# lunarlab-gatech/SLIDE_SLAM

Hardware: AMD Instinct MI355X
Metric: pose-graph updates/sec + ms/Gauss-Newton iter, 8-robot 10k-landmark graph (higher is better)
Workload: dtype f64

## Files before the change

### slide_slam_amd/csrc/chol_kernels.hip

```cpp
#include <hip/hip_runtime.h>
#include <stdlib.h>
#include <algorithm>
#include <type_traits>
#include <utility>
#include <vector>

#include "graph_dev.hpp"
#include "kernels.hpp"

namespace sl {

typedef double v4d __attribute__((ext_vector_type(4)));
constexpr int CHOL_BATCH_MAX = 8;
__device__ inline v4d mfma_f64(double a, double b, v4d c) { return __builtin_amdgcn_mfma_f64_16x16x4f64(a, b, c, 0, 0, 0); }

__device__ inline double rsqrt_nr(double d) {
#ifdef SLIDE_RSQRT_OLD
  double y = __builtin_amdgcn_rsq(d);
  y = y * (1.5 - 0.5 * d * y * y);
  y = y * (1.5 - 0.5 * d * y * y);
  return y;
#else
  double y = __builtin_amdgcn_rsq(d);
  double t = d * y, h = 0.5 * y;
// ... 2182 lines not shown
    if (tid < NB) ys[row] = r0 - ((red[0][row] + red[1][row]) + (red[2][row] + red[3][row]));
  } else {
    acc += __shfl_xor(acc, 1);
    acc += __shfl_xor(acc, 2);
    if (worker && part == 0) ys[i] = r0 - acc;
  }
  __syncthreads();
  if (!worker && has_p) poll(FWD ? c - 1 : c + 1, nloop & 1);
  double z = 0.0;
#pragma unroll
  for (int k = 0; k < 16; ++k) z += mt[k] * ys[16 * part + k];
  z += __shfl_xor(z, 1);
  z += __shfl_xor(z, 2);
  if (has_p) {
    __syncthreads();
    double pv = 0.0;
#pragma unroll
    for (int k = 0; k < 16; ++k) pv += pt[k] * xs[nloop & 1][16 * part + k];
    pv += __shfl_xor(pv, 1);
    pv += __shfl_xor(pv, 2);
    z -= pv;
  }
  if (worker && part == 0) __hip_atomic_store(xout + (size_t)c * NB + i, z, __ATOMIC_RELAXED, __HIP_MEMORY_SCOPE_AGENT);
}
struct ChainBatchArgs {
  int n;
  const double* S[CHOL_BATCH_MAX]; int ld[CHOL_BATCH_MAX]; int T[CHOL_BATCH_MAX];
  const double* ctab[CHOL_BATCH_MAX]; const double* in[CHOL_BATCH_MAX]; double* out[CHOL_BATCH_MAX];
  int* status[CHOL_BATCH_MAX];
  const float* L32[CHOL_BATCH_MAX];
  const int* prof[CHOL_BATCH_MAX];
  const int* first[CHOL_BATCH_MAX];
  double* next_out[CHOL_BATCH_MAX];
  int* next_ticket;
  int Tmax;
};
template <bool FWD, bool F32>
__global__ __launch_bounds__(CHAIN_THREADS) void k_chain_batched(ChainBatchArgs A) {
  __shared__ TabLds W;
  for (;;) {
    const int t = bwd_ticket(&A.status[0][FWD ? 5 : 4]);
    if (t >= A.n * A.Tmax) return;
    const int r = t % A.n, b = t / A.n;
    if (t == 0 && A.next_ticket && threadIdx.x == 0) *A.next_ticket = 0;
    if (b >= A.T[r]) continue;
    tab_chain_body<FWD, F32>(W, A.S[r], A.ld[r], A.T[r], A.L32[r], A.ctab[r], A.in[r], A.out[r], A.status[r], FWD ? b : A.T[r] - 1 - b,
                             A.prof[r], A.first[r], A.next_out[r]);
    return;
  }
}
struct ChainPrepArgs { int n; double* out[CHOL_BATCH_MAX]; int len[CHOL_BATCH_MAX]; int* ticket; };
__global__ void k_chain_prepare(ChainPrepArgs A) {
  const int r = blockIdx.y;
  const int i = blockIdx.x * blockDim.x + threadIdx.x;
  if (r == 0 && i == 0) *A.ticket = 0;
  if (i < A.len[r]) A.out[r][i] = __longlong_as_double((long long)BWD_SENT);
}
static bool chain_has_tables(const CholSystem* d, int n) {
  for (int i = 0; i < n; ++i)
    if (!d[i].L32 || !d[i].ctab) return false;
  return n > 0;
}
void launch_chain_tables(const CholSystem* d, int n, hipStream_t s) {
  if (!chain_has_tables(d, n)) return;
  ChainTabArgs A{};
  A.n = n;
  int Tmax = 0;
  for (int i = 0; i < n; ++i) {
    A.T[i] = d[i].T; A.S[i] = d[i].S; A.ld[i] = d[i].ld; A.Ld[i] = d[i].Ld; A.Winv[i] = d[i].Winv; A.prof[i] = d[i].prof; A.ctab[i] = d[i].ctab;
    Tmax = d[i].T > Tmax ? d[i].T : Tmax;
  }
  if (Tmax > 0) hipLaunchKernelGGL(k_chain_tables, dim3(Tmax, n), dim3(256), 0, s, A);
}
void launch_chain_batch(const CholSystem* d, int n, const double* const* in, double* const* out, bool fwd, bool f32, bool prepared,
                        double* const* next_out, hipStream_t s) {
  ChainBatchArgs A{};
  ChainPrepArgs Pr{};
  A.n = n;
  Pr.n = n;
  int Tmax = 0, total = 0;
  for (int i = 0; i < n; ++i) {
    A.S[i] = d[i].S; A.ld[i] = d[i].ld; A.T[i] = d[i].T; A.ctab[i] = d[i].ctab; A.in[i] = in[i]; A.out[i] = out[i];
    A.status[i] = d[i].status;
    A.L32[i] = d[i].L32;
    A.prof[i] = d[i].prof; A.first[i] = d[i].first;
    Tmax = d[i].T > Tmax ? d[i].T : Tmax;
    total += d[i].T;
    Pr.out[i] = out[i];
    Pr.len[i] = d[i].T * NB;
    A.next_out[i] = next_out ? next_out[i] : nullptr;
  }
  A.next_ticket = next_out ? d[0].status + (fwd ? 4 : 5) : nullptr;
  A.Tmax = Tmax;
  if (total <= 0) return;
  if (!chain_has_tables(d, n)) { fprintf(stderr, "slide_slam_amd: launch_chain_batch without the tables / the packed f32 factor\n"); abort(); }
  Pr.ticket = d[0].status + (fwd ? 5 : 4);
  if (!prepared) hipLaunchKernelGGL(k_chain_prepare, dim3((Tmax * NB + 255) / 256, n), dim3(256), 0, s, Pr);
  if (fwd) {
    if (f32) hipLaunchKernelGGL((k_chain_batched<true, true>), dim3(total), dim3(CHAIN_THREADS), 0, s, A);
    else hipLaunchKernelGGL((k_chain_batched<true, false>), dim3(total), dim3(CHAIN_THREADS), 0, s, A);
  } else {
    if (f32) hipLaunchKernelGGL((k_chain_batched<false, true>), dim3(total), dim3(CHAIN_THREADS), 0, s, A);
    else hipLaunchKernelGGL((k_chain_batched<false, false>), dim3(total), dim3(CHAIN_THREADS), 0, s, A);
  }
}

__global__ __launch_bounds__(256) void k_cov_fwd(const double* __restrict__ S, int ld, int k, const double* __restrict__ Ldk,
                                                 const double* __restrict__ Wk, double* __restrict__ Y, int nT) {
  __shared__ double yk[6][NB];
  __shared__ double xk[6][NB];
  const int tid = threadIdx.x;
  for (int e = tid; e < 6 * NB; e += 256) yk[e / NB][e % NB] = Y[(size_t)(e / NB) * nT + (size_t)k * NB + e % NB];
  __syncthreads();
  const int c = tid >> 4, r = tid & 15;
#pragma unroll 1
  for (int b = 0; b < 4; ++b) {
    if (c < 6) {
      double s = 0.0;
#pragma unroll
      for (int j = 0; j < 16; ++j) s += Wk[(size_t)b * 256 + j * 16 + r] * yk[c][16 * b + j];
      xk[c][16 * b + r] = s;
    }
    __syncthreads();
    for (int e = tid; e < 6 * 16 * (3 - b); e += 256) {
      const int cc = e / (16 * (3 - b)), m = 16 * (b + 1) + e % (16 * (3 - b));
      double s = 0.0;
#pragma unroll
      for (int n = 0; n < 16; ++n) s += Ldk[(size_t)(16 * b + n) * NB + m] * xk[cc][16 * b + n];
      yk[cc][m] -= s;
    }
    __syncthreads();
  }
  if (blockIdx.x == 0) {
    for (int e = tid; e < 6 * NB; e += 256) Y[(size_t)(e / NB) * nT + (size_t)k * NB + e % NB] = xk[e / NB][e % NB];
    return;
  }
  const int i = k + (int)blockIdx.x;
  const double* tile = S + (size_t)(k * NB) * ld + (size_t)i * NB;
  for (int e = tid; e < 6 * NB; e += 256) {
    const int cc = e / NB, row = e % NB;
    double s = 0.0;
#pragma unroll 8
    for (int q = 0; q < NB; ++q) s += tile[(size_t)q * ld + row] * xk[cc][q];
    Y[(size_t)cc * nT + (size_t)i * NB + row] -= s;
  }
}
__global__ __launch_bounds__(256) void k_cov_gram(const double* __restrict__ Y, int nT, int row0, double* __restrict__ cov36) {
  __shared__ double part[36][257];
  const int tid = threadIdx.x;
  double acc[36];
#pragma unroll
  for (int e = 0; e < 36; ++e) acc[e] = 0.0;
  for (int row = row0 + tid; row < nT; row += 256) {
    double y[6];
#pragma unroll
    for (int c = 0; c < 6; ++c) y[c] = Y[(size_t)c * nT + row];
#pragma unroll
    for (int a = 0; a < 6; ++a)
#pragma unroll
      for (int b = 0; b < 6; ++b) acc[6 * a + b] += y[a] * y[b];
  }
#pragma unroll
  for (int e = 0; e < 36; ++e) part[e][tid] = acc[e];
  __syncthreads();
  if (tid < 36) {
    double s = 0.0;
    for (int q = 0; q < 256; ++q) s += part[tid][q];
    cov36[tid] = s;
  }
}
void launch_pose_covariance(const double* S, int ld, int T, const double* Ld, const double* Winv, double* Y, int row0, double* cov36,
                            hipStream_t s) {
  const int nT = T * NB;
  for (int k = row0 / NB; k < T; ++k)
    hipLaunchKernelGGL(k_cov_fwd, dim3((unsigned)(T - k)), dim3(256), 0, s, S, ld, k, Ld + (size_t)k * NB * NB, Winv + (size_t)k * 1024, Y, nT);
  hipLaunchKernelGGL(k_cov_gram, dim3(1), dim3(256), 0, s, Y, nT, row0 / NB * NB, cov36);
}

struct SyrkArgs {
  int n;
  const double* S[CHOL_BATCH_MAX]; int ld[CHOL_BATCH_MAX]; int T[CHOL_BATCH_MAX]; int nbr[CHOL_BATCH_MAX];
  int b0[CHOL_BATCH_MAX];
  double* bord[CHOL_BATCH_MAX]; int ldb[CHOL_BATCH_MAX]; const int* bfirst[CHOL_BATCH_MAX];
  const double* bsrc[CHOL_BATCH_MAX];
  int ks; double* scratch;
  size_t scratch_stride;
  int ks_sys[4];
  double* scratch2; size_t scratch_stride2;
  const int* jobs;
  const int* segtab[CHOL_BATCH_MAX];
};
template <int RD>
__device__ __forceinline__ void border_syrk_body(const SyrkArgs& A) {
  int r = A.ks > 1 ? 0 : blockIdx.z, ib = blockIdx.x, jb = blockIdx.y;
  const int q = A.ks > 1 ? blockIdx.z : 0;
  if (A.jobs) {
    const int j = A.jobs[blockIdx.x];
    r = j >> 20; ib = (j >> 10) & 1023; jb = j & 1023;
  }
  const int nbr = A.nbr[r];
  if (ib > nbr || jb >= nbr || ib < jb) return;
  const int T = A.T[r], ld = A.ld[r];
  int ldb = A.ldb[r];
  int c0 = 0, c1 = T;
  const int* st = A.segtab[r];
  const int nseg = st ? st[0] : 1;
  if (!st && A.bfirst[r]) c0 = max(A.bfirst[r][ib], A.bfirst[r][jb]);
  int ksr = A.ks;
  if (A.ks > 1) {
    if (A.scratch_stride && r < 4 && A.ks_sys[r] > 0) ksr = A.ks_sys[r];
    if (q >= ksr) return;
    const int len = (T - c0 + ksr - 1) / ksr;
    c0 += q * len;
    c1 = min(T, c0 + len);
  }
  const double* bsrc = A.bsrc[r];
  if (!st && c0 >= c1 && !(bsrc && q == 0)) return;
  const double* S = A.S[r];
  const int wq = threadIdx.x >> 6, lane = threadIdx.x & 63, lr = lane & 15, lk = lane >> 4;
  const int ch = (wq >> 1) & 1, rh = wq & 1;
  if (A.jobs && ib == nbr && rh == 1 && !bsrc) return;
  const int B0 = A.b0[r];
  const double* pj0 = S + (size_t)lk * ld + (size_t)(B0 + jb) * NB + 32 * ch + 2 * lr;
  const double* pi0 = S + (size_t)lk * ld + (size_t)(B0 + ib) * NB + 32 * rh + 2 * lr;
  double* cbh = A.bord[r] + (size_t)(jb * NB + 32 * ch + 2 * lk) * ldb + (size_t)ib * NB + 32 * rh + 2 * lr;
  const double* cin = bsrc ? bsrc + (size_t)(jb * NB + 32 * ch + 2 * lk) * ldb + (size_t)ib * NB + 32 * rh + 2 * lr : cbh;
  const int ldin = ldb;
  if (q > 0) {
    ldb = NB;
    double* sc = r < 2 ? A.scratch + (size_t)r * A.scratch_stride : A.scratch2 + (size_t)(r - 2) * A.scratch_stride2;
    cbh = sc + ((size_t)(jb * (nbr + 1) + ib) * (ksr - 1) + (q - 1)) * (NB * NB) + (size_t)(32 * ch + 2 * lk) * NB + 32 * rh + 2 * lr;
  }
  int total = 0;
  if (st) {
    for (int sg = 0; sg < nseg; ++sg) {
      const int* sf = st + 1 + nseg + sg * (nbr + 1);
      const int a0 = max(sf[ib], sf[jb]), a1 = st[1 + sg];
      if (a0 < a1) total += (a1 - a0) * 16;
    }
  } else {
    total = c1 > c0 ? (c1 - c0) * 16 : 0;
  }
  int sg_next = 0, rem = 0, issued = 0;
  const double *lpj = pj0, *lpi = pi0;
  v2d pa[RD], pb[RD];
  auto issue = [&](v2d& ra, v2d& rb) {
    while (rem == 0 && sg_next < nseg) {
      int a0 = c0, a1 = c1;
      if (st) {
        const int* sf = st + 1 + nseg + sg_next * (nbr + 1);
        a0 = max(sf[ib], sf[jb]);
        a1 = st[1 + sg_next];
      }
      ++sg_next;
      if (a0 < a1) {
        rem = (a1 - a0) * 16;
        lpj = pj0 + (size_t)a0 * NB * ld;
        lpi = pi0 + (size_t)a0 * NB * ld;
      }
    }
    ra = *(const v2d*)lpj;
    rb = *(const v2d*)lpi;
    lpj += (size_t)4 * ld;
    lpi += (size_t)4 * ld;
    --rem;
    ++issued;
  };
#pragma unroll
  for (int pre = 0; pre < RD - 1; ++pre)
    if (issued < total) issue(pa[pre], pb[pre]);
  v4d acc[2][2];
#pragma unroll
  for (int a = 0; a < 2; ++a)
#pragma unroll
    for (int e = 0; e < 4; ++e) {
      v2d c2;
      c2[0] = 0.0; c2[1] = 0.0;
      if (q == 0) c2 = *(const v2d*)(cin + (size_t)(8 * e + a) * ldin);
      acc[a][0][e] = c2[0]; acc[a][1][e] = c2[1];
    }
  for (int ks0 = 0; ks0 < total; ks0 += RD) {
#pragma unroll
    for (int u = 0; u < RD; ++u) {
      if (issued < total) issue(pa[(u + RD - 1) % RD], pb[(u + RD - 1) % RD]);
      __builtin_amdgcn_sched_barrier(0);
#pragma unroll
      for (int a = 0; a < 2; ++a) {
        const double na = -pa[u][a];
#pragma unroll
        for (int b = 0; b < 2; ++b) acc[a][b] = mfma_f64(na, pb[u][b], acc[a][b]);
      }
      __builtin_amdgcn_sched_barrier(0);
    }
  }
#pragma unroll
  for (int a = 0; a < 2; ++a)
#pragma unroll
    for (int e = 0; e < 4; ++e) {
      v2d c2;
      c2[0] = acc[a][0][e]; c2[1] = acc[a][1][e];
      *(v2d*)(cbh + (size_t)(8 * e + a) * ldb) = c2;
    }
}
__global__ __launch_bounds__(256) void k_border_syrk(SyrkArgs A) { border_syrk_body<16>(A); }
__global__ __launch_bounds__(256) void k_border_syrk_rd8(SyrkArgs A) { border_syrk_body<8>(A); }
__global__ __launch_bounds__(256) void k_border_syrk_rd4(SyrkArgs A) { border_syrk_body<4>(A); }
static void launch_syrk_kernel(dim3 grid, size_t lds, hipStream_t s, const SyrkArgs& A) {
  static const int rd = getenv("SLIDE_SYRK_RD") ? atoi(getenv("SLIDE_SYRK_RD")) : 16;
  if (rd == 4) hipLaunchKernelGGL(k_border_syrk_rd4, grid, dim3(256), lds, s, A);
  else if (rd == 8) hipLaunchKernelGGL(k_border_syrk_rd8, grid, dim3(256), lds, s, A);
  else hipLaunchKernelGGL(k_border_syrk, grid, dim3(256), lds, s, A);
}
template <int N>
__device__ __forceinline__ void border_reduce_elems(double* __restrict__ bord, int ldb, int nbr, int ks, const double* __restrict__ scratch,
                                                    const int* __restrict__ bfirst, int T, int ib, int jb, int e0, int stride) {
  if (ib > nbr || jb >= nbr || ib < jb) return;
  int c0 = 0;
  if (bfirst) c0 = max(bfirst[ib], bfirst[jb]);
  const int len = (T - c0 + ks - 1) / ks;
  double* dst[N];
  double v[N];
#pragma unroll
  for (int u = 0; u < N; ++u) {
    const int e = e0 + u * stride;
    const int col = e / NB, row = e - col * NB;
    dst[u] = bord + (size_t)(jb * NB + col) * ldb + (size_t)ib * NB + row;
    v[u] = *dst[u];
  }
  int nq = ks;
  while (nq > 1 && c0 + (nq - 1) * len >= T) --nq;
  const double* sq = scratch + (size_t)(jb * (nbr + 1) + ib) * (ks - 1) * (NB * NB) + e0;
  int q = 1;
  for (; q + 1 < nq; q += 2) {
    double p[N], p2[N];
#pragma unroll
    for (int u = 0; u < N; ++u) { p[u] = sq[(size_t)(q - 1) * (NB * NB) + u * stride]; p2[u] = sq[(size_t)q * (NB * NB) + u * stride]; }
#pragma unroll
    for (int u = 0; u < N; ++u) { v[u] += p[u]; v[u] += p2[u]; }
  }
  if (q < nq) {
    double p[N];
#pragma unroll
    for (int u = 0; u < N; ++u) p[u] = sq[(size_t)(q - 1) * (NB * NB) + u * stride];
#pragma unroll
    for (int u = 0; u < N; ++u) v[u] += p[u];
  }
#pragma unroll
  for (int u = 0; u < N; ++u) *dst[u] = v[u];
}
__global__ __launch_bounds__(256) void k_border_syrk_reduce(double* __restrict__ bord, int ldb, int nbr, int ks, const double* __restrict__ scratch,
                                                            const int* __restrict__ bfirst, int T) {
  border_reduce_elems<1>(bord, ldb, nbr, ks, scratch, bfirst, T, blockIdx.x >> 4, blockIdx.y, (blockIdx.x & 15) * 256 + threadIdx.x, 0);
}
__device__ __forceinline__ void border_reduce2_elem(double* __restrict__ bordA, int ldbA, const double* __restrict__ bordB, int ldbB, int nbr,
                                                    int ksA, int ksB, const double* __restrict__ scratchA, const double* __restrict__ scratchB,
                                                    int TA, int TB, int ib, int jb, int e) {
  if (ib > nbr || jb >= nbr || ib < jb) return;
  const int col = e / NB, row = e - col * NB;
  double* dst = bordA + (size_t)(jb * NB + col) * ldbA + (size_t)ib * NB + row;
  double va = *dst, vb = bordB[(size_t)(jb * NB + col) * ldbB + (size_t)ib * NB + row];
  const int lenA = (TA + ksA - 1) / ksA, lenB = (TB + ksB - 1) / ksB;
  for (int q = 1; q < ksA; ++q)
    if (q * lenA < TA) va += scratchA[((size_t)(jb * (nbr + 1) + ib) * (ksA - 1) + (q - 1)) * (NB * NB) + (size_t)col * NB + row];
  for (int q = 1; q < ksB; ++q)
    if (q * lenB < TB) vb += scratchB[((size_t)(jb * (nbr + 1) + ib) * (ksB - 1) + (q - 1)) * (NB * NB) + (size_t)col * NB + row];
  *dst = va + vb;
}
__global__ __launch_bounds__(256) void k_border_syrk_reduce2(double* __restrict__ bordA, int ldbA, const double* __restrict__ bordB, int ldbB, int nbr,
                                                             int ksA, int ksB, const double* __restrict__ scratchA, const double* __restrict__ scratchB,
                                                             int TA, int TB) {
  border_reduce2_elem(bordA, ldbA, bordB, ldbB, nbr, ksA, ksB, scratchA, scratchB, TA, TB, blockIdx.x >> 4, blockIdx.y,
                      (blockIdx.x & 15) * 256 + threadIdx.x);
}
struct Reduce2Pair { double* bordA; const double* bordB; const double* scratchA; const double* scratchB; int ldbA, ldbB, nbr, jb_end, ksA, ksB, TA, TB; };
struct Reduce2Args { Reduce2Pair p[2]; };
__global__ __launch_bounds__(256) void k_border_syrk_reduce2p(Reduce2Args A) {
  const Reduce2Pair& P = A.p[blockIdx.z];
  if ((int)blockIdx.y >= P.jb_end) return;
  border_reduce2_elem(P.bordA, P.ldbA, P.bordB, P.ldbB, P.nbr, P.ksA, P.ksB, P.scratchA, P.scratchB, P.TA, P.TB, blockIdx.x >> 4, blockIdx.y,
                      (blockIdx.x & 15) * 256 + threadIdx.x);
}
union LamSolveLds { ALds a; ChainLds c; };
__global__ __launch_bounds__(512) void k_lam_solve1(double* bord, int ks, const double* __restrict__ scratch, int Tsum, int lam, double* S,
                                                    double* Ld, double* Winv, double* yv, double* dp, int* status, int* ctr) {
  __shared__ LamSolveLds U;
  constexpr int ld = 2 * NB;
  const int tid = threadIdx.x;
  if (ks > 1) border_reduce_elems<16>(bord, ld, 1, ks, scratch, nullptr, Tsum, tid >> 8, 0, tid & 255, 256);
  __syncthreads();
  if (tid < 7 * (NB + 1)) lam_prepare_elems<10>(bord, 1, lam, S, tid % (NB + 1), tid / (NB + 1), 7);
  if (tid == 0) ctr[1] = 0;
  __syncthreads();
  step_type_a(S, ld, 0, 1, 1, 0, -1, Ld, Winv, status, U.a, nullptr, 0, 0);
  __syncthreads();
  extract_y_elem(S, ld, 1, 1, yv, dp, status, nullptr, tid);
  __syncthreads();
  if (tid == 0) status[4] = 1;
  bwd_chain_body<false>(U.c, S, ld, 1, Ld, Winv, yv, dp, status, 0, nullptr, nullptr);
}
void launch_lam_solve1(double* bord, int ks, const double* scratch, int Tsum, int lam, double* S, double* Ld, double* Winv, double* yv, double* dp,
                       int* status, int* ctr, hipStream_t s) {
  hipLaunchKernelGGL(k_lam_solve1, dim3(1), dim3(512), 0, s, bord, scratch ? ks : 1, scratch, Tsum, lam, S, Ld, Winv, yv, dp, status, ctr);
}
LamFuse lam_fuse_env() {
  LamFuse F{3};
  if (const char* e = getenv("SLIDE_LAM_FUSE")) F.mask = atoi(e);
  return F;
}
void launch_border_syrk(const CholSystem* d, int n, hipStream_t s, double* scratch, int ks, bool reduce) {
  SyrkArgs A{};
  A.n = n;
  int nb = 0;
  for (int i = 0; i < n; ++i) {
    A.S[i] = d[i].S; A.ld[i] = d[i].ld; A.T[i] = d[i].T; A.nbr[i] = d[i].nbr; A.bord[i] = d[i].bord; A.ldb[i] = d[i].ldb; A.bfirst[i] = d[i].bfirst; A.bsrc[i] = d[i].bord_src;
    A.segtab[i] = d[i].segtab; A.b0[i] = d[i].b0 > 0 ? d[i].b0 : d[i].T;
    nb = d[i].nbr > nb ? d[i].nbr : nb;
  }
  if (nb <= 0) return;
  if (scratch && n == 1 && ks > 1) {
    A.ks = ks; A.scratch = scratch;
    launch_syrk_kernel(dim3(nb + 1, nb, ks), 0, s, A);
    if (reduce) hipLaunchKernelGGL(k_border_syrk_reduce, dim3(16 * (nb + 1), nb), dim3(256), 0, s, d[0].bord, d[0].ldb, d[0].nbr, ks, scratch, d[0].bfirst, d[0].T);
    return;
  }
  A.ks = 1; A.scratch = nullptr;
  launch_syrk_kernel(dim3(nb + 1, nb, n), 0, s, A);
}
void launch_border_syrk_jobs(const CholSystem* d, int n, const int* jobs, int njobs, int lds_pad, hipStream_t s, double* scratch, int ks, int jb_end,
                             const int* ks_sys, bool fuse_add) {
  SyrkArgs A{};
  A.n = n;
  for (int i = 0; i < n; ++i) {
    A.S[i] = d[i].S; A.ld[i] = d[i].ld; A.T[i] = d[i].T; A.nbr[i] = d[i].nbr; A.bord[i] = d[i].bord; A.ldb[i] = d[i].ldb; A.bfirst[i] = d[i].bfirst; A.bsrc[i] = d[i].bord_src;
    A.segtab[i] = d[i].segtab; A.b0[i] = d[i].b0 > 0 ? d[i].b0 : d[i].T;
  }
  if (njobs <= 0) return;
  A.ks = 1; A.scratch = nullptr; A.jobs = jobs;
  if (scratch && n == 2 && fuse_add && d[0].nbr == d[1].nbr && !d[0].bfirst && !d[1].bfirst) {
    const int nb = d[0].nbr;
    const int ka = std::max(1, ks_sys ? ks_sys[0] : ks), kb = std::max(1, ks_sys ? ks_sys[1] : ks), km = std::max(ka, kb);
    A.ks = km; A.scratch = scratch; A.scratch_stride = std::max<size_t>(1, (size_t)(nb + 1) * nb * (km - 1) * NB * NB);
    A.ks_sys[0] = ka; A.ks_sys[1] = kb;
    launch_syrk_kernel(dim3(njobs, 1, km), lds_pad, s, A);
    hipLaunchKernelGGL(k_border_syrk_reduce2, dim3(16 * (nb + 1), jb_end >= 0 ? jb_end : nb), dim3(256), 0, s, d[0].bord, d[0].ldb, d[1].bord, d[1].ldb, nb,
                       ka, kb, scratch, scratch + A.scratch_stride, d[0].T, d[1].T);
    return;
  }
  if (scratch && n == 1 && ks > 1) {
    A.ks = ks; A.scratch = scratch;
    launch_syrk_kernel(dim3(njobs, 1, ks), lds_pad, s, A);
    const int nb = d[0].nbr;
    hipLaunchKernelGGL(k_border_syrk_reduce, dim3(16 * (nb + 1), jb_end >= 0 ? jb_end : nb), dim3(256), 0, s, d[0].bord, d[0].ldb, nb, ks, scratch, d[0].bfirst, d[0].T);
    return;
  }
  launch_syrk_kernel(dim3(njobs), lds_pad, s, A);
}
void launch_border_syrk_pairs(const CholSystem* top, const CholSystem* lam, const int* jobs, int njobs, hipStream_t s, double* scratch_top,
                              int ks_top, int jb_end, double* scratch_lam, const int* ks_lam) {
  if (njobs <= 0) return;
  SyrkArgs A{};
  A.n = 4;
  for (int i = 0; i < 4; ++i) {
    const CholSystem& d = i < 2 ? top[i] : lam[i - 2];
    A.S[i] = d.S; A.ld[i] = d.ld; A.T[i] = d.T; A.nbr[i] = d.nbr; A.bord[i] = d.bord; A.ldb[i] = d.ldb; A.bfirst[i] = d.bfirst; A.bsrc[i] = d.bord_src;
    A.segtab[i] = d.segtab; A.b0[i] = d.b0 > 0 ? d.b0 : d.T;
  }
  A.jobs = jobs;
  const int nbt = top[0].nbr, nbl = lam[0].nbr;
  const int kt = std::max(1, ks_top), ka = std::max(1, ks_lam[0]), kb = std::max(1, ks_lam[1]), kl = std::max(ka, kb), km = std::max(kt, kl);
  A.ks = km;
  A.scratch = scratch_top; A.scratch_stride = std::max<size_t>(1, (size_t)(nbt + 1) * nbt * (kt - 1) * NB * NB);
  A.scratch2 = scratch_lam; A.scratch_stride2 = std::max<size_t>(1, (size_t)(nbl + 1) * nbl * (kl - 1) * NB * NB);
  A.ks_sys[0] = A.ks_sys[1] = kt; A.ks_sys[2] = ka; A.ks_sys[3] = kb;
  launch_syrk_kernel(dim3(njobs, 1, km), 0, s, A);
  Reduce2Args R{};
  R.p[0] = {top[0].bord, top[1].bord, scratch_top, scratch_top + A.scratch_stride, top[0].ldb, top[1].ldb, nbt, jb_end, kt, kt, top[0].T, top[1].T};
  R.p[1] = {lam[0].bord, lam[1].bord, scratch_lam, scratch_lam + A.scratch_stride2, lam[0].ldb, lam[1].ldb, nbl, nbl, ka, kb, lam[0].T, lam[1].T};
  hipLaunchKernelGGL(k_border_syrk_reduce2p, dim3(16 * (std::max(nbt, nbl) + 1), std::max(jb_end, nbl), 2), dim3(256), 0, s, R);
}
struct BorderApplyArgs {
  int n;
  const double* S[CHOL_BATCH_MAX]; int ld[CHOL_BATCH_MAX]; int T[CHOL_BATCH_MAX]; int nbr[CHOL_BATCH_MAX]; int b0[CHOL_BATCH_MAX];
  double* yv[CHOL_BATCH_MAX]; const double* x[CHOL_BATCH_MAX];
  const int* segtab[CHOL_BATCH_MAX];
};
__global__ __launch_bounds__(256) void k_border_apply(BorderApplyArgs A) {
  const int r = blockIdx.z;
  const int col = blockIdx.x * 4 + (threadIdx.x >> 6), lane = threadIdx.x & 63;
  if (col >= A.T[r] * NB) return;
  const int nrow = A.nbr[r] * NB;
  const double* w = A.S[r] + (size_t)col * A.ld[r] + (size_t)A.b0[r] * NB;
  const double* x = A.x[r];
  double acc = 0.0;
  const int* st = A.segtab[r];
  const int* msk = st ? st + 1 + st[0] + st[0] * (A.nbr[r] + 1) : nullptr;
  if (msk && msk[0] > 0) {
    const int c = col / NB;
    unsigned long long m = (unsigned long long)(unsigned)msk[1 + 2 * c] | ((unsigned long long)(unsigned)msk[2 + 2 * c] << 32);
    while (m) {
      const int t = __ffsll((long long)m) - 1;
      m &= m - 1;
      acc += w[t * NB + lane] * x[t * NB + lane];
    }
  } else {
    for (int q = lane; q < nrow; q += 64) acc += w[q] * x[q];
  }
#pragma unroll
  for (int m = 32; m >= 1; m >>= 1) acc += __shfl_xor(acc, m);
  if (lane == 0) A.yv[r][col] -= acc;
}
void launch_border_apply(const CholSystem* d, int n, const double* const* xloc, hipStream_t s) {
  BorderApplyArgs A{};
  A.n = n;
  int Tmax = 0;
  for (int i = 0; i < n; ++i) {
    A.S[i] = d[i].S; A.ld[i] = d[i].ld; A.T[i] = d[i].T; A.nbr[i] = d[i].nbr; A.yv[i] = d[i].yv; A.x[i] = xloc[i];
    A.b0[i] = d[i].b0 > 0 ? d[i].b0 : d[i].T;
    A.segtab[i] = d[i].segtab;
    Tmax = d[i].T > Tmax ? d[i].T : Tmax;
  }
  if (Tmax > 0) hipLaunchKernelGGL(k_border_apply, dim3(Tmax * NB / 4, 1, n), dim3(256), 0, s, A);
}

void launch_chol_bwd_all(const double* S, int ld, int T, const double* Ld, const double* Winv, double* yv, double* dp,
                         int* status, const int* prof, hipStream_t s, const double* wf_prev, double wf_thr, int wf_Tprev, int wf_lim);
void launch_chol_extract_y(const double* S, int ld, int T, double* yv, double* dp, int* status, hipStream_t s, int nbr, int b0, double* prev) {
  hipLaunchKernelGGL(k_chol_extract_y, dim3((T * NB + 255) / 256), dim3(256), 0, s, S, ld, T, (b0 > 0 ? b0 : T) + nbr, yv, dp, status, prev);
}
struct StepPlan { int kb, nP, g0, g1, nX, TvA, TvB, TvX, nbA, nbB, nbX; long long nA, nB; };
int chol_device_cus() {
  static int n_cu = 0;
  if (!n_cu) {
    int dev = 0;
    hipDeviceProp_t pr;
    if (hipGetDevice(&dev) == hipSuccess && hipGetDeviceProperties(&pr, dev) == hipSuccess) n_cu = pr.multiProcessorCount;
    if (n_cu <= 0) n_cu = 256;
  }
  return n_cu;
}
static thread_local CholPlanHook* t_plan_hook = nullptr;
CholPlanHook::CholPlanHook(int n_cu_, bool dry_) : n_cu(n_cu_), dry(dry_), prev(t_plan_hook) { t_plan_hook = this; }
CholPlanHook::~CholPlanHook() { t_plan_hook = prev; }
static int chol_n_cu() { return (t_plan_hook && t_plan_hook->n_cu > 0) ? t_plan_hook->n_cu : chol_device_cus(); }
static bool chol_hook_launch(int k, int a_split, int a_joins, long long nAw, long long nB) {
  CholPlanHook* h = t_plan_hook;
  if (!h) return false;
  h->trace.insert(h->trace.end(), {k, a_split, a_joins, (int)nAw, (int)nB});
  return h->dry;
}
static StepPlan plan_step(int k, int T, const int* prof, int nbr = 0, const int* bfirst = nullptr, int kofs = 0) {
  static const double frac = getenv("SLIDE_CHOL_FRAC") ? atof(getenv("SLIDE_CHOL_FRAC")) : 0.5;
  StepPlan p{};
  p.kb = k & ~1;
  p.TvA = p.TvB = p.TvX = T;
  if (prof && k < T) {
    p.TvA = prof[k] + 1;
    if (p.kb >= 1) p.TvB = prof[p.kb - 1] + 1;
    if (k >= 1) p.TvX = prof[k - 1] + 1;
  }
  auto active = [&](int upto) { int c = 0; while (c < nbr && (!bfirst || bfirst[c] <= upto + kofs)) ++c; return c; };
  p.nbA = active(k); p.nbB = active(p.kb - 1); p.nbX = active(k - 1);
  p.nA = k < T ? p.TvA - k + p.nbA : 0;
  if (k >= 2 && k < T) {
    p.nP = p.TvB + p.nbB > p.kb ? (p.TvB + p.nbB - p.kb + 1) / 2 : 0;
    long long nG = (long long)p.nP * (p.nP + 1) / 2;
    if (nbr > 0) {
      const int ncol = p.TvB - 1 >= p.kb + 1 ? (p.TvB - 2 - p.kb) / 2 + 1 : 0;
      long long nv = 0;
      for (int bj = 0; bj < ncol && bj < p.nP; ++bj) nv += p.nP - bj;
      nG = nv;
    }
    long long first = (long long)(frac * (double)nG + 0.5);
    if (first < p.nP) first = p.nP;
    if (first > nG) first = nG;
    if (k & 1) { p.g0 = (int)(2 * first); p.g1 = (int)(2 * nG); } else { p.g0 = 0; p.g1 = (int)(2 * first); }
  }
  p.nX = (k & 1) && k + 1 < p.TvX ? (p.TvX + p.nbX - k + 1) / 2 : 0;
  p.nB = p.g1 - p.g0 + p.nX;
  return p;
}
void launch_chol_step(double* S, int ld, int k, int T, double* Ld, double* Winv, int* status, int* ctr, float* L32, const int* h_prof,
                      hipStream_t s, int nbr) {
  const int n_cu = chol_n_cu();
  const StepPlan p = plan_step(k, T, h_prof, nbr, nullptr);
  const long long nA = p.nA, nB = p.nB;
  static const int split_pct = getenv("SLIDE_CHOL_ASPLIT") ? atoi(getenv("SLIDE_CHOL_ASPLIT")) : 100;
  const int a_split = (k > 0 && (2 * nA + nB) * 100 <= (long long)n_cu * split_pct) ? 1 : 0;
  const long long nAw = nA << a_split;
  const long long extra = nB < n_cu ? nB : n_cu;
  const long long free_cu = n_cu - nAw > 8 ? n_cu - nAw : 8;
  static const int join_mul = getenv("SLIDE_CHOL_JOIN") ? atoi(getenv("SLIDE_CHOL_JOIN")) : 1;
  const int a_joins = nB > join_mul * free_cu ? 1 : 0;
  hipLaunchKernelGGL(k_chol_step, dim3((unsigned)(nAw + extra)), dim3(512), 0, s, S, ld, k, T, Ld, Winv, status, ctr, p.kb, p.nP,
                     p.g0, p.g1, p.nX, a_joins, a_split, L32, p.TvA, p.TvB, p.TvX, nbr, p.nbA, p.nbB, p.nbX);
}
struct PairPlan { int ncols, Tv0, Tv1, nb0, nb1, TvB, nbB, nP; long long nA, nB; };
static PairPlan plan_pair(int k, int T, const int* prof, int nbr, const int* bfirst, int kofs) {
  PairPlan p{};
  p.ncols = T - k >= 2 ? 2 : (T - k == 1 ? 1 : 0);
  if (p.ncols == 0) return p;
  auto active = [&](int upto) { int c = 0; while (c < nbr && (!bfirst || bfirst[c] <= upto + kofs)) ++c; return c; };
  p.Tv0 = prof ? prof[k] + 1 : T;
  p.Tv1 = p.ncols == 2 ? (prof ? prof[k + 1] + 1 : T) : p.Tv0;
  p.nb0 = active(k);
  p.nb1 = p.ncols == 2 ? active(k + 1) : p.nb0;
  const int TvL = p.ncols == 2 ? p.Tv1 : p.Tv0, nbL = p.ncols == 2 ? p.nb1 : p.nb0;
  p.nA = (long long)(TvL - (k + p.ncols)) + nbL + 1;
  if (k >= 2) {
    const int kbE = k + 1;
    p.TvB = prof ? prof[k - 1] + 1 : T;
    p.nbB = active(k - 1);
    p.nP = p.TvB + p.nbB > kbE ? (p.TvB + p.nbB - kbE + 1) / 2 : 0;
    long long nG = (long long)p.nP * (p.nP + 1) / 2;
    if (nbr > 0) {
// ... 370 lines not shown
```

Measured before the change: 4167.

## Add LDS-staged async-load ring variant of border SYRK with grid-size dispatch

Adds a border SYRK kernel that streams S panels into a shared-memory ring buffer using global_load_lds direct-to-LDS loads. It uses explicit vmcnt waits and barriers so loads for upcoming k-groups overlap the MFMA accumulation of the current group. A heuristic picks this staged kernel only for certain grid sizes (mid-sized grids, or small split-k grids) and otherwise falls back to the existing register-prefetch kernel. The aim is to hide global memory latency in the SYRK update, at the cost of LDS use, extra barriers and a heuristic that may misjudge some shapes.

Result: no change. 4177, median of 6 (+0.2%).

```diff
diff --git a/slide_slam_amd/csrc/chol_kernels.hip b/slide_slam_amd/csrc/chol_kernels.hip
--- a/slide_slam_amd/csrc/chol_kernels.hip
+++ b/slide_slam_amd/csrc/chol_kernels.hip
@@ -2508,14 +2508,175 @@
       *(v2d*)(cbh + (size_t)(8 * e + a) * ldb) = c2;
     }
 }
-__global__ __launch_bounds__(256) void k_border_syrk(SyrkArgs A) { border_syrk_body<16>(A); }
+__device__ __forceinline__ void syrk_wait_vm(int n) {
+  if (n >= 8) asm volatile("s_waitcnt vmcnt(8)" ::: "memory");
+  else if (n >= 4) asm volatile("s_waitcnt vmcnt(4)" ::: "memory");
+  else if (n >= 2) asm volatile("s_waitcnt vmcnt(2)" ::: "memory");
+  else if (n >= 1) asm volatile("s_waitcnt vmcnt(1)" ::: "memory");
+  else asm volatile("s_waitcnt vmcnt(0)" ::: "memory");
+}
+template <int GK, int D>
+__device__ __forceinline__ void border_syrk_staged_body(const SyrkArgs& A) {
+  static_assert(GK % 2 == 0 && 16 % GK == 0 && D >= 2 && (D - 1) * GK <= 12, "group: an even divisor of 16 k-steps; ring: within syrk_wait_vm's counts");
+  constexpr int KSLAB = 4 * NB / 2;
+  constexpr int SLOT = 2 * GK * KSLAB;
+  __shared__ v2d ring[D * SLOT];
+  int r = A.ks > 1 ? 0 : blockIdx.z, ib = blockIdx.x, jb = blockIdx.y;
+  const int q = A.ks > 1 ? blockIdx.z : 0;
+  if (A.jobs) {
+    const int j = A.jobs[blockIdx.x];
+    r = j >> 20; ib = (j >> 10) & 1023; jb = j & 1023;
+  }
+  const int nbr = A.nbr[r];
+  if (ib > nbr || jb >= nbr || ib < jb) return;
+  const int T = A.T[r], ld = A.ld[r];
+  int ldb = A.ldb[r];
+  int c0 = 0, c1 = T;
+  const int* st = A.segtab[r];
+  const int nseg = st ? st[0] : 1;
+  if (!st && A.bfirst[r]) c0 = max(A.bfirst[r][ib], A.bfirst[r][jb]);
+  int ksr = A.ks;
+  if (A.ks > 1) {
+    if (A.scratch_stride && r < 4 && A.ks_sys[r] > 0) ksr = A.ks_sys[r];
+    if (q >= ksr) return;
+    const int len = (T - c0 + ksr - 1) / ksr;
+    c0 += q * len;
+    c1 = min(T, c0 + len);
+  }
+  const double* bsrc = A.bsrc[r];
+  if (!st && c0 >= c1 && !(bsrc && q == 0)) return;
+  const double* S = A.S[r];
+  const int wq = threadIdx.x >> 6, lane = threadIdx.x & 63, lr = lane & 15, lk = lane >> 4;
+  const int ch = (wq >> 1) & 1, rh = wq & 1;
+  const bool idle = A.jobs && ib == nbr && rh == 1 && !bsrc;
+  const bool diag = ib == jb;
+  const int B0 = A.b0[r];
+  double* cbh = A.bord[r] + (size_t)(jb * NB + 32 * ch + 2 * lk) * ldb + (size_t)ib * NB + 32 * rh + 2 * lr;
+  const double* cin = bsrc ? bsrc + (size_t)(jb * NB + 32 * ch + 2 * lk) * ldb + (size_t)ib * NB + 32 * rh + 2 * lr : cbh;
+  const int ldin = ldb;
+  if (q > 0) {
+    ldb = NB;
+    double* sc = r < 2 ? A.scratch + (size_t)r * A.scratch_stride : A.scratch2 + (size_t)(r - 2) * A.scratch_stride2;
+    cbh = sc + ((size_t)(jb * (nbr + 1) + ib) * (ksr - 1) + (q - 1)) * (NB * NB) + (size_t)(32 * ch + 2 * lk) * NB + 32 * rh + 2 * lr;
+  }
+  int total = 0;
+  if (st) {
+    for (int sg = 0; sg < nseg; ++sg) {
+      const int* sf = st + 1 + nseg + sg * (nbr + 1);
+      const int a0 = max(sf[ib], sf[jb]), a1 = st[1 + sg];
+      if (a0 < a1) total += (a1 - a0) * 16;
+    }
+  } else {
+    total = c1 > c0 ? (c1 - c0) * 16 : 0;
+  }
+  const int ngroups = total / GK;
+  const double* sj0 = S + (size_t)(lane >> 5) * ld + (size_t)(B0 + jb) * NB + 2 * (lane & 31);
+  const double* si0 = S + (size_t)(lane >> 5) * ld + (size_t)(B0 + ib) * NB + 2 * (lane & 31);
+  const double *lsj = sj0, *lsi = si0;
+  int sg_next = 0, rem = 0;
+  const int __attribute__((address_space(4)))* stc = (const int __attribute__((address_space(4)))*)st;
+  auto stage = [&](int slot) {
+    while (rem == 0 && sg_next < nseg) {
+      int a0 = c0, a1 = c1;
+      if (st) {
+        const int __attribute__((address_space(4)))* sf = stc + 1 + nseg + sg_next * (nbr + 1);
+        a0 = max(sf[ib], sf[jb]);
+        a1 = stc[1 + sg_next];
+      }
+      ++sg_next;
+      if (a0 < a1) {
+        rem = (a1 - a0) * 16;
+        lsj = sj0 + (size_t)a0 * NB * ld;
+        lsi = si0 + (size_t)a0 * NB * ld;
+      }
+    }
+    v2d* dst = ring + slot * SLOT + wq * (KSLAB / 2);
+#pragma unroll
+    for (int i = 0; i < GK / 2; ++i)
+      __builtin_amdgcn_global_load_lds((const __attribute__((address_space(1))) void*)(lsj + (size_t)(2 * wq + 8 * i) * ld),
+                                       (__attribute__((address_space(3))) void*)(dst + 4 * i * (KSLAB / 2)), 16, 0, 0);
+    if (!diag) {
+#pragma unroll
+      for (int i = 0; i < GK / 2; ++i)
+        __builtin_amdgcn_global_load_lds((const __attribute__((address_space(1))) void*)(lsi + (size_t)(2 * wq + 8 * i) * ld),
+                                         (__attribute__((address_space(3))) void*)(dst + GK * KSLAB + 4 * i * (KSLAB / 2)), 16, 0, 0);
+    }
+    lsj += (size_t)4 * GK * ld;
+    lsi += (size_t)4 * GK * ld;
+    rem -= GK;
+  };
+  const int nI = diag ? GK / 2 : GK;
+  for (int pre = 0; pre < D - 1; ++pre)
+    if (pre < ngroups) stage(pre);
+  v4d acc[2][2];
+#pragma unroll
+  for (int a = 0; a < 2; ++a)
+#pragma unroll
+    for (int e = 0; e < 4; ++e) { acc[a][0][e] = 0.0; acc[a][1][e] = 0.0; }
+  if (!idle && q == 0) {
+#pragma unroll
+    for (int a = 0; a < 2; ++a)
+#pragma unroll
+      for (int e = 0; e < 4; ++e) {
+        const v2d c2 = *(const v2d*)(cin + (size_t)(8 * e + a) * ldin);
+        acc[a][0][e] = c2[0]; acc[a][1][e] = c2[1];
+      }
+  }
+  const v2d* ra = ring + lk * (KSLAB / 4) + ch * (KSLAB / 8) + lr;
+  const v2d* rb = ring + (diag ? 0 : GK * KSLAB) + lk * (KSLAB / 4) + rh * (KSLAB / 8) + lr;
+  int slot = 0;
+  for (int g = 0; g < ngroups; ++g) {
+    syrk_wait_vm((min(ngroups, g + D - 1) - (g + 1)) * nI);
+    asm volatile("s_waitcnt lgkmcnt(0)" ::: "memory");
+    __builtin_amdgcn_s_barrier();
+    if (g + D - 1 < ngroups) stage(slot == 0 ? D - 1 : slot - 1);
+    if (!idle) {
+      v2d pa[GK], pb[GK];
+#pragma unroll
+      for (int u = 0; u < GK; ++u) {
+        pa[u] = ra[slot * SLOT + u * KSLAB];
+        pb[u] = rb[slot * SLOT + u * KSLAB];
+      }
+      __builtin_amdgcn_sched_barrier(0);
+#pragma unroll
+      for (int u = 0; u < GK; ++u) {
+#pragma unroll
+        for (int a = 0; a < 2; ++a) {
+          const double na = -pa[u][a];
+#pragma unroll
+          for (int b = 0; b < 2; ++b) acc[a][b] = mfma_f64(na, pb[u][b], acc[a][b]);
+        }
+      }
+    }
+    slot = slot + 1 == D ? 0 : slot + 1;
+  }
+  if (idle) return;
+#pragma unroll
+  for (int a = 0; a < 2; ++a)
+#pragma unroll
+    for (int e = 0; e < 4; ++e) {
+      v2d c2;
+      c2[0] = acc[a][0][e]; c2[1] = acc[a][1][e];
+      *(v2d*)(cbh + (size_t)(8 * e + a) * ldb) = c2;
+    }
+}
+__global__ __launch_bounds__(256) void k_border_syrk(SyrkArgs A) { border_syrk_staged_body<4, 2>(A); }
+__global__ __launch_bounds__(256) void k_border_syrk_rd16(SyrkArgs A) { border_syrk_body<16>(A); }
 __global__ __launch_bounds__(256) void k_border_syrk_rd8(SyrkArgs A) { border_syrk_body<8>(A); }
 __global__ __launch_bounds__(256) void k_border_syrk_rd4(SyrkArgs A) { border_syrk_body<4>(A); }
+static bool syrk_staged_wins(dim3 grid) {
+  const size_t wg = (size_t)grid.x * grid.y * grid.z;
+  constexpr size_t CUS = 256;
+  if (grid.z > 1) return wg <= 64;
+  return wg > 2 * CUS && wg <= 6 * CUS;
+}
 static void launch_syrk_kernel(dim3 grid, size_t lds, hipStream_t s, const SyrkArgs& A) {
-  static const int rd = getenv("SLIDE_SYRK_RD") ? atoi(getenv("SLIDE_SYRK_RD")) : 16;
+  static const int rd = getenv("SLIDE_SYRK_RD") ? atoi(getenv("SLIDE_SYRK_RD")) : 0;
+  static const int stage = getenv("SLIDE_SYRK_STAGE") ? atoi(getenv("SLIDE_SYRK_STAGE")) : -1;
   if (rd == 4) hipLaunchKernelGGL(k_border_syrk_rd4, grid, dim3(256), lds, s, A);
   else if (rd == 8) hipLaunchKernelGGL(k_border_syrk_rd8, grid, dim3(256), lds, s, A);
-  else hipLaunchKernelGGL(k_border_syrk, grid, dim3(256), lds, s, A);
+  else if (rd != 16 && (stage == 1 || (stage < 0 && syrk_staged_wins(grid)))) hipLaunchKernelGGL(k_border_syrk, grid, dim3(256), lds, s, A);
+  else hipLaunchKernelGGL(k_border_syrk_rd16, grid, dim3(256), lds, s, A);
 }
 template <int N>
 __device__ __forceinline__ void border_reduce_elems(double* __restrict__ bord, int ldb, int nbr, int ks, const double* __restrict__ scratch,
```
